# IntelLabs/GKL

Measured on AMD Instinct MI355X. Metric: pairhmm_gcups, higher is better.
Workload: dtype f32

## Files before the change

### gkl_amd/csrc/pairhmm_api.hip

```cpp
#include <hip/hip_runtime.h>
#include <unistd.h>
#include <rccl/rccl.h>
#include <dlfcn.h>

#include <algorithm>
#include <atomic>
#include <cmath>
#include <cstdarg>
#include <cstdio>
#include <cstdlib>
#include <chrono>
#include <condition_variable>
#include <functional>
#include <cstring>
#include <limits>
#include <memory>
#include <mutex>
#include <new>
#include <string>
#include <thread>
#include <deque>
#include <type_traits>
#include <vector>

// ... 353 lines not shown
  static const bool v = server_socket_from_env() != nullptr;
  return v;
}

void* gklhip_host_alloc(size_t bytes) {
  if (client_process()) return malloc(bytes ? bytes : 1);
  void* p = nullptr;
  if (hipHostMalloc(&p, bytes ? bytes : 1, hipHostMallocDefault | hipHostMallocPortable) != hipSuccess) {
    (void)hipGetLastError();
    return nullptr;
  }
  return p;
}

void gklhip_host_free(void* p) {
  if (client_process()) { free(p); return; }
  if (p) (void)hipHostFree(p);
}

static int get_step_times_impl(gklhip_ctx* ctx, int32_t steps_back, float* ms_main, float* ms_fallback, float* ms_total) {
  if (!ctx) return fail(GKLHIP_ERR_INVALID_ARG, "context is NULL");
  if (ctx->remote) return fail(GKLHIP_ERR_UNSUPPORTED, "gklhip_get_step_times: not available on a client context of the PairHMM server");
  std::lock_guard<std::mutex> lock(ctx->mu);
  DevCtx* c = ctx->dev[0];
  if (c->cfg.record_events != 2) return fail(GKLHIP_ERR_INVALID_ARG, "context was not created with record_events = 2");
  if (steps_back < 0 || steps_back >= DevCtx::kEventRing || steps_back >= c->calls)
    return fail(GKLHIP_ERR_INVALID_ARG, "steps_back %d outside the %d recorded calls", steps_back,
                (int)std::min<int64_t>(c->calls, DevCtx::kEventRing));
  HIP_TRY(hipSetDevice(c->device));
  const int slot = (int)((c->calls - 1 - steps_back) % DevCtx::kEventRing);
  hipEvent_t* e = c->ev_ring[slot];
  HIP_TRY(hipEventSynchronize(e[5]));
  float ms = 0;
  HIP_TRY(hipEventElapsedTime(&ms, e[1], e[2])); if (ms_main) *ms_main = ms;
  HIP_TRY(hipEventElapsedTime(&ms, e[3], e[4])); if (ms_fallback) *ms_fallback = c->ring_double[slot] ? 0.f : ms;
  HIP_TRY(hipEventElapsedTime(&ms, e[0], e[5])); if (ms_total) *ms_total = ms;
  return GKLHIP_OK;
}

int gklhip_get_stats(gklhip_ctx* c, gklhip_stats* out) {
  if (!c || !out) return fail(GKLHIP_ERR_INVALID_ARG, "NULL argument");
  std::lock_guard<std::mutex> lock(c->mu);
  *out = c->stats;
  return GKLHIP_OK;
}

static int get_raw_impl(gklhip_ctx* ctx, float* raw32, double* raw64, uint8_t* used64) {
  if (!ctx) return fail(GKLHIP_ERR_INVALID_ARG, "context is NULL");
  if (ctx->remote) return fail(GKLHIP_ERR_UNSUPPORTED, "gklhip_get_raw: the raw sums stay on the PairHMM server (client context)");
  std::lock_guard<std::mutex> lock(ctx->mu);
  int64_t n_fallback = 0;
  bool any = false;
  const std::vector<DevCtx*>& list = ctx->last ? *ctx->last : ctx->dev;
  for (size_t d = 0; d < list.size(); d++) {
    DevCtx* c = list[d];
    if (list.size() > 1 && ctx->bounds[d + 1] == ctx->bounds[d]) continue;
    if (!c->have_last) continue;
    any = true;
    HIP_TRY(hipSetDevice(c->device));
    hipStream_t s = c->last_stream;
    const size_t n = (size_t)c->last_pairs;
    const size_t at = (size_t)ctx->bounds[d] * (size_t)ctx->last_haps;
    if (raw32 && !c->cfg.use_double) HIP_TRY(hipMemcpyAsync(raw32 + at, c->raw32.p, n * 4, hipMemcpyDeviceToHost, s));
    if (raw64) HIP_TRY(hipMemcpyAsync(raw64 + at, c->raw64.p, n * 8, hipMemcpyDeviceToHost, s));
    if (used64) HIP_TRY(hipMemcpyAsync(used64 + at, c->used64.p, n, hipMemcpyDeviceToHost, s));
    int32_t cnt[2] = {0, 0};
    HIP_TRY(hipMemcpyAsync(cnt, c->counters.p, 8, hipMemcpyDeviceToHost, s));
    HIP_TRY(hipStreamSynchronize(s));
    c->stats.n_fallback = c->cfg.use_double ? (int64_t)n : cnt[0];
    n_fallback += c->stats.n_fallback;
  }
  if (!any) return fail(GKLHIP_ERR_INVALID_ARG, "no completed call to read back");
  ctx->stats.n_fallback = n_fallback;
  HIP_TRY(hipSetDevice(ctx->dev[0]->device));
  return GKLHIP_OK;
}

int gklhip_plan_describe(int32_t n_reads, int32_t n_haps, const int64_t* read_off, const int64_t* hap_off,
                         int32_t rows_per_lane, int32_t* lanes_out, int64_t lanes_cap, int32_t* n_groups_out,
                         int32_t* n_long_out) {
  if (n_reads < 0 || n_haps < 0 || !read_off || !hap_off || (rows_per_lane != 4 && rows_per_lane != 8))
    return -fail(GKLHIP_ERR_INVALID_ARG, "bad arguments to gklhip_plan_describe");
  Plan p;
  build_plan(n_reads, n_haps, read_off, hap_off, rows_per_lane, kTargetCols, &p, true);
  if (n_groups_out) *n_groups_out = (int32_t)p.groups.size();
  if (n_long_out) *n_long_out = (int32_t)p.long_reads.size();
  if (lanes_out) {
    const int64_t n = std::min<int64_t>(lanes_cap, (int64_t)p.lanes.size());
    for (int64_t i = 0; i < n; i++) { lanes_out[2 * i] = p.lanes[i].read; lanes_out[2 * i + 1] = p.lanes[i].block; }
  }
  return p.n_chunks;
}

int64_t gklhip_get_table_f32(int which, float* dst, int64_t cap) {
  const HostTables<float>& t = host_tables_f32();
  const std::vector<float>* v = which == 0 ? &t.ph2pr : which == 1 ? &t.mm : which == 2 ? &t.div3 : nullptr;
  if (!v) return -1;
  if (dst) memcpy(dst, v->data(), sizeof(float) * (size_t)std::min<int64_t>(cap, (int64_t)v->size()));
  return (int64_t)v->size();
}
int64_t gklhip_get_table_f64(int which, double* dst, int64_t cap) {
  const HostTables<double>& t = host_tables_f64();
  const std::vector<double>* v = which == 0 ? &t.ph2pr : which == 1 ? &t.mm : which == 2 ? &t.div3 : nullptr;
  if (!v) return -1;
  if (dst) memcpy(dst, v->data(), sizeof(double) * (size_t)std::min<int64_t>(cap, (int64_t)v->size()));
  return (int64_t)v->size();
}

#include "pairhmm_diagnostics.h"

int gklhip_init_devices(const gklhip_config* cfg, const int32_t* devices, int32_t n_devices, gklhip_ctx** out_ctx) { return guarded([&] { return init_devices_impl(cfg, devices, n_devices, out_ctx); }); }
int gklhip_compute_device(gklhip_ctx* c, const gklhip_batch* dev_batch, double* out_dev, void* hip_stream) { return guarded([&] { return compute_device_impl(c, dev_batch, out_dev, hip_stream); }); }
int gklhip_compute(gklhip_ctx* c, const gklhip_batch* hb, double* out_host) { return guarded([&] { return compute_impl(c, hb, out_host); }); }
int gklhip_get_raw(gklhip_ctx* ctx, float* raw32, double* raw64, uint8_t* used64) { return guarded([&] { return get_raw_impl(ctx, raw32, raw64, used64); }); }
int gklhip_get_step_times(gklhip_ctx* ctx, int32_t steps_back, float* ms_main, float* ms_fallback, float* ms_total) { return guarded([&] { return get_step_times_impl(ctx, steps_back, ms_main, ms_fallback, ms_total); }); }
int gklhip_rccl_selftest(int32_t device) { return guarded([&] { return rccl_selftest_impl(device); }); }
int gklhip_init(const gklhip_config* cfg, gklhip_ctx** out_ctx) { return guarded([&] { return init_impl(cfg, out_ctx); }); }

}
```

### gkl_amd/csrc/pairhmm_ctx.h

```cpp
#pragma once

using namespace gklhip;

namespace {
struct EnvSwitches {
  static bool on_unless_zero(const char* name) { const char* v = getenv(name); return !v || atoi(v) != 0; }
  static int integer(const char* name) { const char* v = getenv(name); return v ? atoi(v) : 0; }
  const bool wide_long = on_unless_zero("GKLHIP_WIDE_LONG");
  const bool super_long = on_unless_zero("GKLHIP_SUPER_LONG");
  const bool fused_pairs = on_unless_zero("GKLHIP_FUSED_PAIRS");
  const int64_t fused_max = [] { const char* v = getenv("GKLHIP_FUSED_MAX_PAIRS"); return v ? atoll(v) : -1LL; }();
  const bool xcd_aware = on_unless_zero("GKLHIP_XCD_AWARE");
  const bool timing = getenv("GKLHIP_TIMING") != nullptr;
  const int combine_load = integer("GKL_HIP_COMBINE_LOAD");
  const int target_cols = integer("GKLHIP_TARGET_COLS");
  const int fb_wanted_jobs = integer("GKLHIP_FB_WANTED_JOBS");
  const int plan_blocks = integer("GKLHIP_PLAN_BLOCKS");
  const int finalize_threads = integer("GKL_HIP_FINALIZE_THREADS");
  const int finalize_min = integer("GKL_HIP_FINALIZE_MIN");
  const bool combine = [] { const char* v = getenv("GKL_HIP_COMBINE"); return !(v && v[0] == '0'); }();
  const bool quiet = getenv("GKL_HIP_QUIET") != nullptr;
  const bool one_device_engine = integer("GKL_HIP_DEVICE_ENGINES") == 1;
};
const EnvSwitches g_env;
// ... 6 lines not shown
  char buf[512];
  va_list ap;
  va_start(ap, fmt);
  vsnprintf(buf, sizeof buf, fmt, ap);
  va_end(ap);
  g_err = buf;
  return status;
}

int fail_noexcept(int status, const char* msg) noexcept {
  try { g_err = msg; } catch (...) {}
  return status;
}
template <typename F>
int guarded(F&& body) noexcept {
  try { return body(); }
  catch (const std::bad_alloc&) { return fail_noexcept(GKLHIP_ERR_OOM, "host memory allocation failed"); }
  catch (const std::exception& e) { return fail_noexcept(GKLHIP_ERR_HIP, e.what()); }
  catch (...) { return fail_noexcept(GKLHIP_ERR_HIP, "unexpected C++ exception"); }
}

#define HIP_TRY(expr)                                                                        \
  do {                                                                                       \
    hipError_t e__ = (expr);                                                                 \
    if (e__ != hipSuccess) {                                                                 \
      (void)hipGetLastError();                                                               \
      return fail(e__ == hipErrorOutOfMemory ? GKLHIP_ERR_OOM : GKLHIP_ERR_HIP, "%s: %s",    \
                  #expr, hipGetErrorString(e__));                                            \
    }                                                                                        \
  } while (0)

constexpr size_t kTrimFloor = (size_t)32 << 20;
constexpr int kTrimCalls = 16;
constexpr int kTrimQuiet = 64;
inline bool trim_due(size_t n, size_t cap, int* small_uses, int* since_grow) {
  if (*since_grow < kTrimQuiet) ++*since_grow;
  if (cap <= kTrimFloor || n >= cap / 4) { *small_uses = 0; return false; }
  if (*small_uses < kTrimCalls) ++*small_uses;
  return *small_uses >= kTrimCalls && *since_grow >= kTrimQuiet;
}
struct DevBuf {
  void* p = nullptr;
  size_t cap = 0;
  int small_uses = 0, since_grow = kTrimQuiet;
  int reserve(size_t n) {
    if (n <= cap && !trim_due(n, cap, &small_uses, &since_grow)) return GKLHIP_OK;
    if (n > cap) since_grow = 0;
    small_uses = 0;
    if (p) { (void)hipFree(p); p = nullptr; cap = 0; }
    const size_t want = n + n / 4 + 256;
    HIP_TRY(hipMalloc(&p, want));
    cap = want;
    return GKLHIP_OK;
  }
  void release() { if (p) (void)hipFree(p); p = nullptr; cap = 0; }
  template <typename T> T* as() const { return static_cast<T*>(p); }
};
struct PinBuf {
  void* p = nullptr;
  size_t cap = 0;
  int small_uses = 0, since_grow = kTrimQuiet;
  int reserve(size_t n) {
    if (n <= cap && !trim_due(n, cap, &small_uses, &since_grow)) return GKLHIP_OK;
    if (n > cap) since_grow = 0;
    small_uses = 0;
    if (p) { (void)hipHostFree(p); p = nullptr; cap = 0; }
    const size_t want = n + n / 4 + 256;
    HIP_TRY(hipHostMalloc(&p, want, hipHostMallocDefault));
    cap = want;
    return GKLHIP_OK;
  }
  void release() { if (p) (void)hipHostFree(p); p = nullptr; cap = 0; }
  template <typename T> T* as() const { return static_cast<T*>(p); }
};
}

struct DevCtx {
  gklhip_config cfg;
  int device = 0;
  int n_cus = 256;
  int n_xcds = 8;
  int asm_general = 1;
  int speculate_fp64 = 0;
  int lds_oob_zero = 1;
  hipStream_t stream = nullptr;
  DevBuf tab32, tab64;
  DevTables<float> dt32;
  DevTables<double> dt64;
  PinBuf stage_slot[2];
  DevBuf plan_dev_slot[2];
  hipEvent_t stage_free_slot[2] = {nullptr, nullptr};
  hipEvent_t plan_unused_slot[2] = {nullptr, nullptr};
  hipStream_t upload_stream = nullptr;
  bool upload_eager = false;
  hipStream_t pad_stream = nullptr;
  int plan_slot = 0;
  DevBuf raw32, raw64, used64, counters, stream_buf, out_dev;
  DevBuf lanes_main;
  DevBuf read_fail, lanes2, jobs, jobs_long, fail_order, fail_hist, hap_flags;
  DevBuf batch_dev;
  PinBuf res_pin;
  WorkerPool workers;
  hipStream_t copy_stream = nullptr;
  hipEvent_t policy_done = nullptr, early_copy_done = nullptr;
  hipEvent_t call_done = nullptr;
  bool have_call_done = false;
  static constexpr int kEventRing = 64;
  hipEvent_t ev_ring[kEventRing][6] = {};
  hipEvent_t* ev = ev_ring[0];
  int64_t calls = 0;
  bool ring_double[kEventRing] = {};
  gklhip_stats stats;
  int64_t last_pairs = 0;
  hipStream_t last_stream = nullptr;
  bool have_last = false;
  Plan plan;
  std::vector<PlanLane> long_lanes;
  std::vector<FwdJob> long_jobs;
  std::vector<int64_t> sub_read_off;
  DevBuf carry;
};
```

### gkl_amd/csrc/pairhmm_ctx_lifecycle.h

```cpp
#pragma once

namespace {

std::atomic<int> g_eager_upload_holders{0};

int trim_streams(DevCtx* c) {
  if (!c->copy_stream && !c->pad_stream && (!c->upload_stream || c->upload_eager)) return 0;
  (void)hipSetDevice(c->device);
  for (hipStream_t s : {c->stream, c->copy_stream, c->upload_stream, c->have_last ? c->last_stream : nullptr})
    if (s && hipStreamQuery(s) != hipSuccess) { (void)hipGetLastError(); return 0; }
  int n = 0;
  if (c->copy_stream) { (void)hipStreamDestroy(c->copy_stream); c->copy_stream = nullptr; n++; }
  if (c->pad_stream) { (void)hipStreamDestroy(c->pad_stream); c->pad_stream = nullptr; n++; }
  if (c->upload_stream && !c->upload_eager) { (void)hipStreamDestroy(c->upload_stream); c->upload_stream = nullptr; n++; }
  return n;
}

void dev_done(DevCtx* c) {
  if (!c) return;
  (void)hipSetDevice(c->device);
  if (c->upload_eager) g_eager_upload_holders--;
  if (c->stream) (void)hipStreamSynchronize(c->stream);
  if (c->last_stream && c->have_last) (void)hipStreamSynchronize(c->last_stream);
  for (DevBuf* b : {&c->tab32, &c->tab64, &c->plan_dev_slot[0], &c->plan_dev_slot[1], &c->raw32, &c->raw64, &c->used64,
// ... 4 lines not shown
  c->stage_slot[1].release();
  c->res_pin.release();
  if (c->policy_done) (void)hipEventDestroy(c->policy_done);
  if (c->early_copy_done) (void)hipEventDestroy(c->early_copy_done);
  if (c->call_done) (void)hipEventDestroy(c->call_done);
  if (c->copy_stream) { (void)hipStreamSynchronize(c->copy_stream); (void)hipStreamDestroy(c->copy_stream); }
  for (auto& set : c->ev_ring)
    for (auto& e : set) if (e) (void)hipEventDestroy(e);
  for (int k = 0; k < 2; k++) {
    if (c->stage_free_slot[k]) (void)hipEventDestroy(c->stage_free_slot[k]);
    if (c->plan_unused_slot[k]) (void)hipEventDestroy(c->plan_unused_slot[k]);
  }
  if (c->upload_stream) { (void)hipStreamSynchronize(c->upload_stream); (void)hipStreamDestroy(c->upload_stream); }
  if (c->pad_stream) (void)hipStreamDestroy(c->pad_stream);
  if (c->stream) (void)hipStreamDestroy(c->stream);
  delete c;
}

int dev_init(const gklhip_config& cfg, int dev, int ndev, DevCtx** out) {
  *out = nullptr;
  if (dev < 0 || dev >= ndev) return fail(GKLHIP_ERR_INVALID_ARG, "device %d of %d", dev, ndev);
  HIP_TRY(hipSetDevice(dev));
  {
    static const char* sched = getenv("GKL_HIP_SCHEDULE");
    if (sched && *sched) {
      const unsigned f = strcmp(sched, "yield") == 0 ? hipDeviceScheduleYield : strcmp(sched, "blocking") == 0 ? hipDeviceScheduleBlockingSync
                         : strcmp(sched, "spin") == 0 ? hipDeviceScheduleSpin : hipDeviceScheduleAuto;
      (void)hipSetDeviceFlags(f);
      (void)hipGetLastError();
    }
  }
  hipDeviceProp_t prop;
  HIP_TRY(hipGetDeviceProperties(&prop, dev));
  if (strncmp(prop.gcnArchName, "gfx950", 6) != 0)
    return fail(GKLHIP_ERR_NO_DEVICE, "device %d is %s; this library is built for gfx950 only", dev, prop.gcnArchName);
  DevCtx* c = new (std::nothrow) DevCtx();
  if (!c) return fail(GKLHIP_ERR_OOM, "context allocation failed");
  c->cfg = cfg;
  c->device = dev;
  c->n_cus = std::max(1, prop.multiProcessorCount);
  {
    int xccs = 0;
    if (hipDeviceGetAttribute(&xccs, hipDeviceAttributeNumberOfXccs, dev) != hipSuccess) { (void)hipGetLastError(); xccs = 8; }
    c->n_xcds = std::max(1, std::min(xccs, 64));
  }
  memset(&c->stats, 0, sizeof c->stats);
  int rc = GKLHIP_OK;
  auto bail = [&](int status) { dev_done(c); return status; };
  if (hipStreamCreateWithFlags(&c->stream, hipStreamNonBlocking) != hipSuccess) return bail(fail(GKLHIP_ERR_HIP, "hipStreamCreate failed"));
  {
    static std::mutex mu;
    static std::vector<int> checked;
    std::lock_guard<std::mutex> l(mu);
    if ((int)checked.size() <= dev) checked.resize((size_t)dev + 1, 0);
    static std::vector<int> oob_checked;
    if ((int)oob_checked.size() <= dev) oob_checked.resize((size_t)dev + 1, 0);
    if (checked[(size_t)dev] == 0 || oob_checked[(size_t)dev] == 0) {
      uint32_t* d_out = nullptr;
      uint32_t h_out[3] = {1u, 1u, 1u};
      if (hipMalloc(reinterpret_cast<void**>(&d_out), 12) != hipSuccess) return bail(fail(GKLHIP_ERR_OOM, "hipMalloc failed"));
      float f_den; double d_den;
      { const uint32_t fb = 1u; memcpy(&f_den, &fb, 4); const uint64_t db = 0x0000000100000001ull; memcpy(&d_den, &db, 8); }
      bool ok = hipMemsetAsync(d_out, 0, 12, c->stream) == hipSuccess;
      hipLaunchKernelGGL(flush_selftest_kernel, dim3(1), dim3(1), 0, c->stream, d_out, f_den, d_den);
      hipLaunchKernelGGL(lds_oob_selftest_kernel, dim3(1024), dim3(256), 0, c->stream, d_out + 2);
      hipLaunchKernelGGL((lds_oob_selftest_big_kernel<78 * 256, 512>), dim3(4 * 2 * (unsigned)c->n_cus), dim3(512), 0, c->stream, d_out + 2);
      hipLaunchKernelGGL((lds_oob_selftest_big_kernel<128 * 256, 256>), dim3(4 * (unsigned)c->n_cus), dim3(256), 0, c->stream, d_out + 2);
      ok = ok && hipGetLastError() == hipSuccess && hipMemcpyAsync(h_out, d_out, 12, hipMemcpyDeviceToHost, c->stream) == hipSuccess &&
           hipStreamSynchronize(c->stream) == hipSuccess;
      (void)hipFree(d_out);
      if (!ok) { (void)hipGetLastError(); return bail(fail(GKLHIP_ERR_HIP, "the start-up self-tests could not run on device %d", dev)); }
      checked[(size_t)dev] = h_out[0] == 0u && h_out[1] == 0u ? 1 : -1;
      oob_checked[(size_t)dev] = h_out[2] == 0u ? 1 : -1;
      if (oob_checked[(size_t)dev] < 0)
        fprintf(stderr, "[gklhip] pairhmm: LDS reads beyond the allocation do not return 0 on device %d (%08x): the fp32 general steps stay in C++\n", dev, h_out[2]);
    }
    if (checked[(size_t)dev] < 0)
      return bail(fail(GKLHIP_ERR_HIP, "this library was built without the denormal-flush flags its kernels depend on (gkl_amd/csrc/Makefile: HIPFLAGS)"));
    c->lds_oob_zero = oob_checked[(size_t)dev] > 0 ? 1 : 0;
  }
  {
    const char* ag = getenv("GKLHIP_ASM_GENERAL");
    c->asm_general = ag ? (atoi(ag) != 0) : 1;
    const char* sp = getenv("GKLHIP_SPECULATE_FP64");
    c->speculate_fp64 = sp ? (atoi(sp) != 0) : 0;
    const char* sf = getenv("GKLHIP_SELFTEST_FAIL");
    if (sf && strcmp(sf, "lds_oob") == 0) {
      c->lds_oob_zero = 0;
      fprintf(stderr, "[gklhip] pairhmm: GKLHIP_SELFTEST_FAIL=lds_oob: the fp32 general steps stay in C++ for this context\n");
    }
  }
  if (g_eager_upload_holders.fetch_add(1) == 0) {
    if (hipStreamCreateWithFlags(&c->upload_stream, hipStreamNonBlocking) != hipSuccess) { g_eager_upload_holders--; return bail(fail(GKLHIP_ERR_HIP, "hipStreamCreate failed")); }
    c->upload_eager = true;
  } else {
    g_eager_upload_holders--;
  }
  if (const char* v = getenv("GKL_HIP_EAGER_STREAMS")) {
    const int k = atoi(v);
    if (k >= 7) { if (aux_streams(c) != GKLHIP_OK) return bail(GKLHIP_ERR_HIP); }
    else for (int i = 0; i < k; i++) { hipStream_t d = nullptr; (void)hipStreamCreateWithFlags(&d, hipStreamNonBlocking); }
  }
  for (int k = 0; k < 2; k++)
    if (hipEventCreateWithFlags(&c->stage_free_slot[k], hipEventDisableTiming) != hipSuccess ||
        hipEventCreateWithFlags(&c->plan_unused_slot[k], hipEventDisableTiming) != hipSuccess)
      return bail(fail(GKLHIP_ERR_HIP, "hipEventCreate failed"));
  if (hipEventCreateWithFlags(&c->policy_done, hipEventDisableTiming) != hipSuccess ||
      hipEventCreateWithFlags(&c->early_copy_done, hipEventDisableTiming) != hipSuccess ||
      hipEventCreateWithFlags(&c->call_done, hipEventDisableTiming) != hipSuccess)
    return bail(fail(GKLHIP_ERR_HIP, "hipEventCreate failed"));
  for (int k = 0; k < 2; k++)
    if (hipEventRecord(c->stage_free_slot[k], c->stream) != hipSuccess || hipEventRecord(c->plan_unused_slot[k], c->stream) != hipSuccess)
      return bail(fail(GKLHIP_ERR_HIP, "hipEventRecord failed"));
  {
    const int sets = c->cfg.record_events == 2 ? DevCtx::kEventRing : 1;
    for (int k = 0; k < sets; k++)
      for (auto& e : c->ev_ring[k])
        if (hipEventCreate(&e) != hipSuccess) return bail(fail(GKLHIP_ERR_HIP, "hipEventCreate failed"));
  }
  if ((rc = upload_tables(c, host_tables_f32(), &c->tab32, &c->dt32))) return bail(rc);
  if ((rc = upload_tables(c, host_tables_f64(), &c->tab64, &c->dt64))) return bail(rc);
  *out = c;
  return GKLHIP_OK;
}

}
```

### gkl_amd/csrc/pairhmm_device_pass.h

```cpp
#pragma once

namespace {

int aux_streams(DevCtx* c) {
  if (!c->upload_stream) HIP_TRY(hipStreamCreateWithFlags(&c->upload_stream, hipStreamNonBlocking));
  if (!c->copy_stream) {
    HIP_TRY(hipStreamCreateWithFlags(&c->copy_stream, hipStreamNonBlocking));
    if (!c->pad_stream) HIP_TRY(hipStreamCreateWithFlags(&c->pad_stream, hipStreamNonBlocking));
  }
  return GKLHIP_OK;
}

template <typename T>
int upload_tables(DevCtx* c, const HostTables<T>& h, DevBuf* buf, DevTables<T>* dt) {
  const size_t n = (size_t)kQuals * 2 + kMmEntries;
  int st = buf->reserve(n * sizeof(T));
  if (st) return st;
  T* base = buf->as<T>();
  {
    T* pin = nullptr;
    HIP_TRY(hipHostMalloc(reinterpret_cast<void**>(&pin), n * sizeof(T), hipHostMallocDefault));
    memcpy(pin, h.ph2pr.data(), kQuals * sizeof(T));
    memcpy(pin + kQuals, h.div3.data(), kQuals * sizeof(T));
    memcpy(pin + 2 * kQuals, h.mm.data(), kMmEntries * sizeof(T));
// ... 163 lines not shown
    int64_t blocks = 0;
    for (int r = 0; r < n_reads; r++) {
      const int nb = blocks_for((int)(read_off[r + 1] - read_off[r]), rpl);
      if (nb <= kLanes) blocks += nb;
    }
    const int64_t chunks = std::max<int64_t>(1, (blocks + kLanes - 1) / kLanes);
    const int64_t groups = std::min<int64_t>(n_haps, std::max<int64_t>((total_cols + kTargetCols - 1) / kTargetCols,
                                                                        (4096 + chunks - 1) / chunks));
    return chunks * groups;
  };
  if (jobs_at(kRplF32) * load >= 2048 || max_len > 4 * kLanes - 1) return kRplF32;
  if (jobs_at(4) * load >= 1024 || max_len > 2 * kLanes - 1) return 4;
  return 2;
}

void launch_pair_policy_two_step(const FwdArgs<double>& d, const PairPolicyArgs& q, int rows, int fma, int64_t n_pairs, int32_t* list, hipStream_t s) {
  hipLaunchKernelGGL(pairhmm_pair_flag_kernel, dim3((unsigned)((n_pairs + 255) / 256)), dim3(256), 0, s, q, (int32_t)n_pairs, list);
  const dim3 grid((unsigned)std::max<int64_t>(256, n_pairs / 2)), block(64);
  if (fma) {
    if (rows == 2)      hipLaunchKernelGGL((pairhmm_pair_recompute_kernel<2, true>), grid, block, 0, s, d, q, list);
    else if (rows == 4) hipLaunchKernelGGL((pairhmm_pair_recompute_kernel<4, true>), grid, block, 0, s, d, q, list);
    else                hipLaunchKernelGGL((pairhmm_pair_recompute_kernel<kRplF64, true>), grid, block, 0, s, d, q, list);
  } else {
    if (rows == 2)      hipLaunchKernelGGL((pairhmm_pair_recompute_kernel<2, false>), grid, block, 0, s, d, q, list);
    else if (rows == 4) hipLaunchKernelGGL((pairhmm_pair_recompute_kernel<4, false>), grid, block, 0, s, d, q, list);
    else                hipLaunchKernelGGL((pairhmm_pair_recompute_kernel<kRplF64, false>), grid, block, 0, s, d, q, list);
  }
}
void launch_main_f32(const FwdArgs<float>& a, int rpl_main, int fma, int n_blocks, hipStream_t s) {
  if (rpl_main == 2)      launch_stream<float, 2>(a, fma, n_blocks, s);
  else if (rpl_main == 4) launch_stream<float, 4>(a, fma, n_blocks, s);
  else                    launch_stream<float, kRplF32>(a, fma, n_blocks, s);
}
void launch_pair_policy(const FwdArgs<double>& d, const PairPolicyArgs& q, int rows, int fma, int64_t n_pairs, hipStream_t s) {
  const dim3 grid((unsigned)n_pairs), block(64);
  if (fma) {
    if (rows == 2)      hipLaunchKernelGGL((pairhmm_pair_policy_kernel<2, true>), grid, block, 0, s, d, q);
    else if (rows == 4) hipLaunchKernelGGL((pairhmm_pair_policy_kernel<4, true>), grid, block, 0, s, d, q);
    else                hipLaunchKernelGGL((pairhmm_pair_policy_kernel<kRplF64, true>), grid, block, 0, s, d, q);
  } else {
    if (rows == 2)      hipLaunchKernelGGL((pairhmm_pair_policy_kernel<2, false>), grid, block, 0, s, d, q);
    else if (rows == 4) hipLaunchKernelGGL((pairhmm_pair_policy_kernel<4, false>), grid, block, 0, s, d, q);
    else                hipLaunchKernelGGL((pairhmm_pair_policy_kernel<kRplF64, false>), grid, block, 0, s, d, q);
  }
}

void launch_pair_fused(const FwdArgs<float>& f, const FwdArgs<double>& d, const PairPolicyArgs& q, int rows, int fma, int64_t n_pairs,
                       hipStream_t s, bool speculate = false) {
  if (speculate) {
    const dim3 grid((unsigned)n_pairs), block(128);
    if (fma) hipLaunchKernelGGL((pairhmm_pair_spec_kernel<kRplF64, true>), grid, block, 0, s, f, d, q);
    else     hipLaunchKernelGGL((pairhmm_pair_spec_kernel<kRplF64, false>), grid, block, 0, s, f, d, q);
    return;
  }
  const dim3 grid((unsigned)n_pairs), block(64);
  if (rows <= 4) {
    if (fma) hipLaunchKernelGGL((pairhmm_pair_fused_kernel<4, true>), grid, block, 0, s, f, d, q);
    else     hipLaunchKernelGGL((pairhmm_pair_fused_kernel<4, false>), grid, block, 0, s, f, d, q);
    return;
  }
  if (fma) hipLaunchKernelGGL((pairhmm_pair_fused_kernel<kRplF64, true>), grid, block, 0, s, f, d, q);
  else     hipLaunchKernelGGL((pairhmm_pair_fused_kernel<kRplF64, false>), grid, block, 0, s, f, d, q);
}

int run_device(DevCtx* c, const gklhip_batch* db, double* out_dev, int finalize_mode, hipStream_t s, bool inline_host,
               SmallLaunch* defer = nullptr) {
  const int n_reads = db->n_reads, n_haps = db->n_haps;
  const int64_t n_pairs = (int64_t)n_reads * n_haps;
  gklhip_stats& st = c->stats;
  memset(&st, 0, sizeof st);
  st.n_pairs = n_pairs;
  c->have_last = false;
  if (n_pairs == 0) return GKLHIP_OK;
  const bool use_double = c->cfg.use_double != 0;
  const int fma = c->cfg.fma_mode != 0;

  const auto t_plan0 = std::chrono::steady_clock::now();
  Plan& plan = c->plan;
  const int rpl64 = kRplF64Jobs;
  const int load_env = g_env.combine_load;
  const int load = !defer ? 1 : load_env > 0 ? load_env : std::max(1, g_host_calls_in_flight.load(std::memory_order_relaxed) / 2);
  const int rpl_main = use_double ? rpl64 : pick_f32_rpl(c->cfg.rows_per_lane, n_reads, n_haps, db->read_off, db->hap_off, load);
  const int target_cols_env = g_env.target_cols;
  build_plan(n_reads, n_haps, db->read_off, db->hap_off, rpl_main, target_cols_env > 0 ? target_cols_env : kTargetCols, &plan);
  std::vector<PlanLane>& long_lanes = c->long_lanes;
  std::vector<FwdJob>& long_jobs = c->long_jobs;
  long_lanes.clear(); long_jobs.clear();
  const std::vector<int32_t>& long_main = plan.long_reads;
  const int n_long_main = (int)long_main.size();
  for (int32_t r : long_main) { long_lanes.resize(long_lanes.size() + kLanes, PlanLane{-1, 0}); long_lanes[long_lanes.size() - kLanes] = PlanLane{r, 0}; }
  int n_long64 = 0;
  if (!use_double && plan.max_read_len > kLanes * kRplF64Jobs - 1)
    for (int r = 0; r < n_reads; r++)
      if (blocks_for((int)(db->read_off[r + 1] - db->read_off[r]), kRplF64Jobs) > kLanes) {
        long_lanes.resize(long_lanes.size() + kLanes, PlanLane{-1, 0});
        long_lanes[long_lanes.size() - kLanes] = PlanLane{r, 0};
        n_long64++;
      }
  for (int i = 0; i < n_long_main; i++)
    for (const PlanGroup& g : plan.groups) long_jobs.push_back(FwdJob{i, g.hap_begin, g.hap_end, 0});
  int carry_len = 0;
  for (const PlanGroup& g : plan.groups) {
    const int last = g.hap_end - 1;
    carry_len = std::max(carry_len, plan.hap_pos[last] + plan.hap_len[last] - plan.hap_pos[g.hap_begin] + 3 * kLanes);
  }
  carry_len = (carry_len + 63) / 64 * 64;
  const size_t rl = (size_t)db->read_off[n_reads], hl = (size_t)db->hap_off[n_haps];
  const PlanLayout L = layout_for(plan, n_reads, n_haps, long_lanes.size(), long_jobs.size(), inline_host ? rl : 0, inline_host ? hl : 0);

  int rc;
  const int slot = c->plan_slot ^= 1;
  PinBuf& stage = c->stage_slot[slot];
  DevBuf& plan_dev = c->plan_dev_slot[slot];
  HIP_TRY(hipEventSynchronize(c->stage_free_slot[slot]));
  if (L.total > stage.cap || L.total > plan_dev.cap) HIP_TRY(hipEventSynchronize(c->plan_unused_slot[slot]));
  if ((rc = stage.reserve(L.total))) return rc;
  if ((rc = plan_dev.reserve(L.total))) return rc;
  unsigned char* hs = stage.as<unsigned char>();
  memcpy(hs + L.place_chunk, plan.place_chunk.data(), (size_t)n_reads * 4);
  memcpy(hs + L.place_lane, plan.place_lane.data(), (size_t)n_reads);
  memcpy(hs + L.chunk_used, plan.chunk_used.data(), (size_t)plan.n_chunks);
  memcpy(hs + L.groups, plan.groups.data(), plan.groups.size() * sizeof(PlanGroup));
  memcpy(hs + L.hap_len, plan.hap_len.data(), (size_t)n_haps * 4);
  memcpy(hs + L.hap_pos, plan.hap_pos.data(), (size_t)n_haps * 4);
  memcpy(hs + L.hap_pos_flat, plan.hap_pos_flat.data(), (size_t)n_haps * 4);
  memcpy(hs + L.hap_orig, plan.hap_orig.data(), (size_t)n_haps * 4);
  memcpy(hs + L.hap_sidx, plan.hap_sidx.data(), (size_t)n_haps * 4);
  memcpy(hs + L.hap_group, plan.hap_group.data(), (size_t)n_haps * 4);
  memcpy(hs + L.hap_src, plan.hap_src.data(), (size_t)n_haps * 4);
  {
    float* y32 = reinterpret_cast<float*>(hs + L.y0_32);
    double* y64 = reinterpret_cast<double*>(hs + L.y0_64);
    const float i32 = host_tables_f32().initial_constant;
    const double i64 = host_tables_f64().initial_constant;
    for (int k = 0; k < n_haps; k++) {
      y32[k] = i32 / (float)plan.hap_len[k];
      y64[k] = i64 / (double)plan.hap_len[k];
    }
  }
  memcpy(hs + L.read_off, db->read_off, (size_t)(n_reads + 1) * 8);
  if (!long_lanes.empty()) memcpy(hs + L.long_lanes, long_lanes.data(), long_lanes.size() * sizeof(PlanLane));
  if (!long_jobs.empty()) memcpy(hs + L.long_jobs, long_jobs.data(), long_jobs.size() * sizeof(FwdJob));
  {
    int32_t lc[4] = {(int32_t)long_jobs.size(), n_long_main, n_long64, 0};
    memcpy(hs + L.long_count, lc, sizeof lc);
  }
  unsigned char* dp = plan_dev.as<unsigned char>();
  gklhip_batch dbi = *db;
  if (inline_host) {
    const uint8_t* srcs[5] = {db->read_bases, db->read_quals, db->ins_gop, db->del_gop, db->gcp};
    for (int i = 0; i < 5; i++) memcpy(hs + L.batch + i * L.batch_stride, srcs[i], rl);
    memcpy(hs + L.batch + 5 * L.batch_stride, db->hap_bases, hl);
    unsigned char* d = dp + L.batch;
    dbi.read_bases = d; dbi.read_quals = d + L.batch_stride; dbi.ins_gop = d + 2 * L.batch_stride;
    dbi.del_gop = d + 3 * L.batch_stride; dbi.gcp = d + 4 * L.batch_stride; dbi.hap_bases = d + 5 * L.batch_stride;
    uint32_t* sg = reinterpret_cast<uint32_t*>(hs + L.stream);
    uint32_t* sf = reinterpret_cast<uint32_t*>(hs + L.stream_flat);
    uint8_t* hn = hs + L.has_n;
    for (int k = 0; k < n_haps; k++) {
      const uint8_t* src = db->hap_bases + plan.hap_src[k];
      const int len = plan.hap_len[k], pg = plan.hap_pos[k], pf = plan.hap_pos_flat[k];
      bool has_n = false;
      for (int col = 0; col < len; col++) {
        const uint8_t bb = src[col];
        const uint32_t e = bb == 'C' ? 1u : bb == 'T' ? 2u : bb == 'G' ? 3u : bb == 'N' ? 4u : 0u;
        sg[pg + col] = e; sf[pf + col] = e;
        has_n |= bb == 'N';
// ... 349 lines not shown
```

### gkl_amd/csrc/pairhmm_plan.cpp

```cpp
#include "pairhmm_plan.h"

#include <algorithm>
#include <cstdlib>
#include <numeric>

namespace gklhip {

namespace {
constexpr int kLanes = 64;
constexpr int kWantedJobs = 4096;
}

void build_plan(int n_reads, int n_haps, const int64_t* read_off, const int64_t* hap_off,
                int rows_per_lane, int target_cols, Plan* out, bool want_lanes) {
  Plan& p = *out;
  p.rows_per_lane = rows_per_lane;
  p.n_chunks = 0;
  p.n_stream = p.n_stream_flat = 0;
  p.useful_rows = 0;
  p.max_read_len = p.max_hap_len = 0;
  p.groups.clear(); p.long_reads.clear(); p.lanes.clear(); p.chunk_used.clear();

  p.hap_len.resize(n_haps);
  p.hap_pos.resize(n_haps);
  p.hap_pos_flat.resize(n_haps);
  p.hap_orig.resize(n_haps);
  p.hap_sidx.resize(n_haps);
  p.hap_group.resize(n_haps);
  p.hap_src.resize(n_haps);
  int64_t total_cols = 0;
  std::iota(p.hap_orig.begin(), p.hap_orig.end(), 0);
  std::stable_sort(p.hap_orig.begin(), p.hap_orig.end(), [&](int32_t a, int32_t b) {
    return hap_off[a + 1] - hap_off[a] < hap_off[b + 1] - hap_off[b];
  });
  for (int k = 0; k < n_haps; k++) {
    const int h = p.hap_orig[k];
    const int len = (int)(hap_off[h + 1] - hap_off[h]);
    p.hap_len[k] = len;
    p.hap_sidx[h] = k;
    p.max_hap_len = std::max(p.max_hap_len, len);
    total_cols += len + 1;
  }
  if (target_cols < 256) target_cols = 256;
  int n_groups = (int)((total_cols + target_cols - 1) / target_cols);
  bool equal_split = true, graded = false;
  if (rows_per_lane > 0) {
    int64_t blocks = 0;
    {
      int shift = -1;
      for (int b = 0; b < 8; b++) if ((1 << b) == rows_per_lane) shift = b;
      const int long_from = kLanes * rows_per_lane;
      for (int r = 0; r < n_reads; r++) {
        const int R = (int)(read_off[r + 1] - read_off[r]);
        p.max_read_len = std::max(p.max_read_len, R);
        if (R < long_from) blocks += shift >= 0 ? (R + rows_per_lane) >> shift : blocks_for(R, rows_per_lane);
      }
    }
    const int64_t chunks_est = std::max<int64_t>(1, (blocks + kLanes - 1) / kLanes);
    static const int wanted_env = [] { const char* v = getenv("GKLHIP_WANTED_JOBS"); return v ? atoi(v) : 0; }();
    const int64_t slots = kWantedJobs, chunks_hi = chunks_est + chunks_est / 100 + 1;
    const int64_t wanted = wanted_env > 0 ? wanted_env : (chunks_est <= 650 || total_cols <= 4 * (int64_t)target_cols ? 3 * slots : slots);
    int64_t by_jobs = std::min<int64_t>((wanted + chunks_est - 1) / chunks_est, n_haps);
    if (chunks_hi * by_jobs > slots && chunks_hi * by_jobs * 10 <= slots * 13) by_jobs = std::max<int64_t>(1, slots / chunks_hi);
    graded = chunks_hi * by_jobs > slots;
    if (by_jobs >= n_groups) n_groups = (int)by_jobs;
    else equal_split = false;
  }
  n_groups = std::max(1, std::min(n_groups, n_haps));
  std::vector<int64_t> want;
  if (equal_split || total_cols < 3 * (int64_t)target_cols) {
    const int64_t per_group = (total_cols + n_groups - 1) / n_groups;
    want.assign((size_t)n_groups, per_group);
    if (graded && equal_split && n_groups >= 4)
      for (int i = 0; i < n_groups; i++)
        want[(size_t)i] = std::max<int64_t>(1, (int64_t)((double)per_group * (1.35 - 0.7 * (double)i / (double)(n_groups - 1))));
  } else {
    const int64_t tail[4] = {target_cols / 2, target_cols / 4, target_cols / 8, target_cols / 8};
    const int64_t head = total_cols - target_cols;
    const int n_big = (int)std::max<int64_t>(1, (head + target_cols / 2) / target_cols);
    want.assign((size_t)n_big, (head + n_big - 1) / n_big);
    want.insert(want.end(), tail, tail + 4);
  }
  {
    int h = 0;
    size_t gi = 0;
    while (h < n_haps) {
      PlanGroup g;
      g.hap_begin = h;
      g.stream_begin = p.n_stream;
      g.pad_ = 0;
      int64_t cols = 0;
      const bool last = gi + 1 >= want.size();
      const int64_t share = want[std::min(gi, want.size() - 1)];
      do {
        p.hap_pos[h] = p.n_stream;
        p.hap_pos_flat[h] = p.n_stream_flat;
        p.n_stream_flat += p.hap_len[h] + 1;
        p.hap_group[h] = (int32_t)p.groups.size();
        p.hap_src[h] = (int32_t)hap_off[p.hap_orig[h]];
        p.n_stream += p.hap_len[h] + 1;
        cols += p.hap_len[h] + 1;
        h++;
      } while (h < n_haps && (last || cols + (p.hap_len[h] + 1) / 2 < share));
      g.hap_end = h;
      p.n_stream += kLanes;
      p.groups.push_back(g);
      gi++;
    }
  }

  p.n_stream_flat += kLanes;

  if (rows_per_lane <= 0)
    for (int r = 0; r < n_reads; r++)
      p.max_read_len = std::max(p.max_read_len, (int)(read_off[r + 1] - read_off[r]));
  p.place_chunk.resize((size_t)n_reads);
  p.place_lane.resize((size_t)n_reads);
  if (rows_per_lane <= 0 || n_reads == 0) return;
  static thread_local std::vector<int32_t> order;
  static thread_local PackScratch scratch;
  order.clear();
  const int long_from = kLanes * rows_per_lane;
  if (p.max_read_len < long_from) {
    order.resize((size_t)n_reads);
    std::iota(order.begin(), order.end(), 0);
  } else {
    for (int r = 0; r < n_reads; r++) {
      if ((int)(read_off[r + 1] - read_off[r]) < long_from) order.push_back(r);
      else { p.long_reads.push_back(r); p.place_chunk[r] = -1; p.place_lane[r] = 0; }
    }
  }
  p.n_chunks = pack_reads_place(order.data(), (int)order.size(), read_off, rows_per_lane,
                                (int)std::max<size_t>(order.size(), 1), p.place_chunk.data(), p.place_lane.data(),
                                &p.chunk_used, &p.useful_rows, &scratch);
  if (want_lanes) expand_lanes(p, n_reads, read_off, &p.lanes);
}

void expand_lanes(const Plan& p, int n_reads, const int64_t* read_off, std::vector<PlanLane>* lanes) {
  lanes->assign((size_t)p.n_chunks * kLanes, PlanLane{-1, 0});
  for (int r = 0; r < n_reads; r++) {
    if (p.place_chunk[r] < 0) continue;
    const int nb = blocks_for((int)(read_off[r + 1] - read_off[r]), p.rows_per_lane);
    PlanLane* dst = lanes->data() + (size_t)p.place_chunk[r] * kLanes + p.place_lane[r];
    for (int b = 0; b < nb; b++) dst[b] = PlanLane{r, b};
  }
}

int pack_reads_place(const int32_t* order_in, int n, const int64_t* read_off, int rows_per_lane, int window,
                     int32_t* place_chunk, uint8_t* place_lane, std::vector<uint8_t>* chunk_used,
                     int64_t* useful_rows, PackScratch* sc) {
  const int rpl = rows_per_lane;
  if (window < 1) window = 1;
  int shift = -1;
  for (int b = 0; b < 8; b++) if ((1 << b) == rpl) shift = b;
  sc->need_of.resize((size_t)n);
  int64_t rows = 0;
  for (int i = 0; i < n; i++) {
    const int32_t r = order_in[i];
    const int R = (int)(read_off[r + 1] - read_off[r]);
    sc->need_of[i] = (uint8_t)(shift >= 0 ? (R + rpl) >> shift : blocks_for(R, rpl));
    rows += R;
  }
  if (useful_rows) *useful_rows += rows;
  const int wcap = std::min(n, window);
  sc->sorted.resize((size_t)wcap);
  sc->sorted_need.resize((size_t)wcap);
  const uint8_t* need_of = sc->need_of.data();
  int chunks_total = 0;
  for (int w0 = 0; w0 < n; w0 += window) {
    const int cnt = std::min(window, n - w0);
    int32_t bucket[kLanes + 2] = {0};
    for (int i = 0; i < cnt; i++) bucket[need_of[w0 + i]]++;
    int32_t start[kLanes + 2];
    int acc = 0;
    for (int c = kLanes; c >= 1; c--) { start[c] = acc; acc += bucket[c]; }
    for (int i = 0; i < cnt; i++) {
      const int at = start[need_of[w0 + i]]++;
      sc->sorted[at] = order_in[w0 + i];
      sc->sorted_need[at] = need_of[w0 + i];
    }
    int32_t head[kLanes + 1];
    for (int c = 0; c <= kLanes; c++) head[c] = -1;
    uint64_t open_sizes = 0;
    const size_t base = chunk_used->size();
    sc->next.clear();
    for (int i = 0; i < cnt; i++) {
      const int32_t r = sc->sorted[i];
      const int nb = sc->sorted_need[i];
      const uint64_t fits = nb <= 63 ? open_sizes >> (nb - 1) : 0;
      int chunk, c;
      if (!fits) {
        chunk = (int)sc->next.size();
        sc->next.push_back(-1);
        chunk_used->push_back(0);
        c = kLanes;
      } else {
        c = nb + __builtin_ctzll(fits);
        chunk = head[c];
        head[c] = sc->next[chunk];
        if (head[c] < 0) open_sizes &= ~(1ull << (c - 1));
      }
      uint8_t& used = (*chunk_used)[base + (size_t)chunk];
      place_chunk[r] = (int32_t)(base + (size_t)chunk);
      place_lane[r] = used;
      used = (uint8_t)(used + nb);
      const int left = c - nb;
      if (left > 0) { sc->next[chunk] = head[left]; head[left] = chunk; open_sizes |= 1ull << (left - 1); }
    }
    chunks_total += (int)sc->next.size();
  }
  return chunks_total;
}

int pack_reads_windowed(const int32_t* order_in, int n, const int64_t* read_off, int rows_per_lane,
                        int window, std::vector<PlanLane>* lanes, int64_t* useful_rows) {
  const int rpl = rows_per_lane;
  if (window < 1) window = 1;
  int chunks_total = 0;
  int shift = -1;
  for (int b = 0; b < 8; b++) if ((1 << b) == rpl) shift = b;
  std::vector<uint8_t> need_of((size_t)n);
  int64_t need_sum = 0;
  for (int i = 0; i < n; i++) {
    const int32_t r = order_in[i];
    const int R = (int)(read_off[r + 1] - read_off[r]);
    need_of[i] = (uint8_t)(shift >= 0 ? (R + rpl) >> shift : blocks_for(R, rpl));
    need_sum += need_of[i];
    if (useful_rows) *useful_rows += R;
  }
  {
    const size_t want = lanes->size() + (size_t)(need_sum + need_sum / 8 + 2 * kLanes);
    if (lanes->capacity() < want) lanes->reserve(std::max(want, 2 * lanes->capacity()));
  }
  std::vector<int32_t> sorted((size_t)std::min(n, window));
  std::vector<uint8_t> sorted_need((size_t)std::min(n, window));
  std::vector<int32_t> next;
  std::vector<int32_t> used;
  for (int w0 = 0; w0 < n; w0 += window) {
    const int cnt = std::min(window, n - w0);
    int32_t bucket[kLanes + 2] = {0};
    for (int i = 0; i < cnt; i++) bucket[need_of[w0 + i]]++;
    int32_t start[kLanes + 2];
    int acc = 0;
    for (int c = kLanes; c >= 1; c--) { start[c] = acc; acc += bucket[c]; }
    for (int i = 0; i < cnt; i++) {
      const int at = start[need_of[w0 + i]]++;
      sorted[at] = order_in[w0 + i];
      sorted_need[at] = need_of[w0 + i];
    }
    int32_t head[kLanes + 1];
    for (int c = 0; c <= kLanes; c++) head[c] = -1;
    next.clear();
    used.clear();
    const size_t base = lanes->size();
    for (int i = 0; i < cnt; i++) {
      const int32_t r = sorted[i];
      const int nb = sorted_need[i];
      int c = nb;
      while (c <= kLanes && head[c] < 0) c++;
      int chunk;
      if (c > kLanes) {
        chunk = (int)used.size();
        used.push_back(0);
        next.push_back(-1);
        lanes->resize(base + (size_t)(chunk + 1) * kLanes, PlanLane{-1, 0});
        c = kLanes;
      } else {
        chunk = head[c];
        head[c] = next[chunk];
// ... 14 lines not shown
```

### gkl_amd/csrc/pairhmm_plan.h

```cpp
#pragma once
#include <cstdint>
#include <vector>

namespace gklhip {

struct PlanLane {
  int32_t read;
  int32_t block;
};

struct PlanGroup {
  int32_t hap_begin, hap_end, stream_begin, pad_;
};

struct Plan {
  int rows_per_lane = 0;
  int n_chunks = 0;
  std::vector<int32_t> place_chunk;
  std::vector<uint8_t> place_lane;
  std::vector<uint8_t> chunk_used;
  std::vector<PlanLane> lanes;
  std::vector<PlanGroup> groups;
  std::vector<int32_t> hap_len;
  std::vector<int32_t> hap_pos;
  std::vector<int32_t> hap_pos_flat;
  std::vector<int32_t> hap_orig;
  std::vector<int32_t> hap_sidx;
  std::vector<int32_t> hap_group;
  std::vector<int32_t> hap_src;
  int32_t n_stream = 0;
  int32_t n_stream_flat = 0;
  std::vector<int32_t> long_reads;
  int64_t useful_rows = 0;
  int max_read_len = 0;
  int max_hap_len = 0;
};

inline int blocks_for(int R, int rpl) { return (R + rpl) / rpl; }

void build_plan(int n_reads, int n_haps, const int64_t* read_off, const int64_t* hap_off,
                int rows_per_lane, int target_cols, Plan* out, bool want_lanes = false);

void expand_lanes(const Plan& p, int n_reads, const int64_t* read_off, std::vector<PlanLane>* lanes);

int pack_reads_windowed(const int32_t* order, int n, const int64_t* read_off, int rows_per_lane,
                        int window, std::vector<PlanLane>* lanes, int64_t* useful_rows);

struct PackScratch {
  std::vector<uint8_t> need_of, sorted_need;
  std::vector<int32_t> sorted, next;
};
int pack_reads_place(const int32_t* order, int n, const int64_t* read_off, int rows_per_lane, int window,
                     int32_t* place_chunk, uint8_t* place_lane, std::vector<uint8_t>* chunk_used,
                     int64_t* useful_rows, PackScratch* scratch);

}
```

Before: 4761.

## Pack reads into chunks with bounded exact-fill search before best-fit

```diff
diff --git a/gkl_amd/csrc/pairhmm_api.hip b/gkl_amd/csrc/pairhmm_api.hip
--- a/gkl_amd/csrc/pairhmm_api.hip
+++ b/gkl_amd/csrc/pairhmm_api.hip
@@ -459,7 +459,7 @@
   if (n_reads < 0 || n_haps < 0 || !read_off || !hap_off || (rows_per_lane != 4 && rows_per_lane != 8))
     return -fail(GKLHIP_ERR_INVALID_ARG, "bad arguments to gklhip_plan_describe");
   Plan p;
-  build_plan(n_reads, n_haps, read_off, hap_off, rows_per_lane, kTargetCols, &p, true);
+  build_plan(n_reads, n_haps, read_off, hap_off, rows_per_lane, kTargetCols, &p, true, EnvSwitches::on_unless_zero("GKLHIP_EXACT_FIT"));
   if (n_groups_out) *n_groups_out = (int32_t)p.groups.size();
   if (n_long_out) *n_long_out = (int32_t)p.long_reads.size();
   if (lanes_out) {
diff --git a/gkl_amd/csrc/pairhmm_ctx.h b/gkl_amd/csrc/pairhmm_ctx.h
--- a/gkl_amd/csrc/pairhmm_ctx.h
+++ b/gkl_amd/csrc/pairhmm_ctx.h
@@ -112,6 +112,7 @@
   int n_xcds = 8;
   int asm_general = 1;
   int speculate_fp64 = 0;
+  int exact_fit = 1;
   int lds_oob_zero = 1;
   hipStream_t stream = nullptr;
   DevBuf tab32, tab64;
diff --git a/gkl_amd/csrc/pairhmm_ctx_lifecycle.h b/gkl_amd/csrc/pairhmm_ctx_lifecycle.h
--- a/gkl_amd/csrc/pairhmm_ctx_lifecycle.h
+++ b/gkl_amd/csrc/pairhmm_ctx_lifecycle.h
@@ -110,6 +110,7 @@
   {
     const char* ag = getenv("GKLHIP_ASM_GENERAL");
     c->asm_general = ag ? (atoi(ag) != 0) : 1;
+    c->exact_fit = EnvSwitches::on_unless_zero("GKLHIP_EXACT_FIT") ? 1 : 0;
     const char* sp = getenv("GKLHIP_SPECULATE_FP64");
     c->speculate_fp64 = sp ? (atoi(sp) != 0) : 0;
     const char* sf = getenv("GKLHIP_SELFTEST_FAIL");
diff --git a/gkl_amd/csrc/pairhmm_device_pass.h b/gkl_amd/csrc/pairhmm_device_pass.h
--- a/gkl_amd/csrc/pairhmm_device_pass.h
+++ b/gkl_amd/csrc/pairhmm_device_pass.h
@@ -269,7 +269,8 @@
   const int load = !defer ? 1 : load_env > 0 ? load_env : std::max(1, g_host_calls_in_flight.load(std::memory_order_relaxed) / 2);
   const int rpl_main = use_double ? rpl64 : pick_f32_rpl(c->cfg.rows_per_lane, n_reads, n_haps, db->read_off, db->hap_off, load);
   const int target_cols_env = g_env.target_cols;
-  build_plan(n_reads, n_haps, db->read_off, db->hap_off, rpl_main, target_cols_env > 0 ? target_cols_env : kTargetCols, &plan);
+  build_plan(n_reads, n_haps, db->read_off, db->hap_off, rpl_main, target_cols_env > 0 ? target_cols_env : kTargetCols, &plan,
+             false, c->exact_fit != 0);
   std::vector<PlanLane>& long_lanes = c->long_lanes;
   std::vector<FwdJob>& long_jobs = c->long_jobs;
   long_lanes.clear(); long_jobs.clear();
diff --git a/gkl_amd/csrc/pairhmm_plan.cpp b/gkl_amd/csrc/pairhmm_plan.cpp
--- a/gkl_amd/csrc/pairhmm_plan.cpp
+++ b/gkl_amd/csrc/pairhmm_plan.cpp
@@ -12,7 +12,7 @@
 }
 
 void build_plan(int n_reads, int n_haps, const int64_t* read_off, const int64_t* hap_off,
-                int rows_per_lane, int target_cols, Plan* out, bool want_lanes) {
+                int rows_per_lane, int target_cols, Plan* out, bool want_lanes, bool exact_fit) {
   Plan& p = *out;
   p.rows_per_lane = rows_per_lane;
   p.n_chunks = 0;
@@ -132,7 +132,7 @@
   }
   p.n_chunks = pack_reads_place(order.data(), (int)order.size(), read_off, rows_per_lane,
                                 (int)std::max<size_t>(order.size(), 1), p.place_chunk.data(), p.place_lane.data(),
-                                &p.chunk_used, &p.useful_rows, &scratch);
+                                &p.chunk_used, &p.useful_rows, &scratch, exact_fit);
   if (want_lanes) expand_lanes(p, n_reads, read_off, &p.lanes);
 }
 
@@ -146,9 +146,49 @@
   }
 }
 
+namespace {
+
+bool exact_fill(int32_t* left, uint64_t* avail, int s, int mx, int* budget, uint8_t* picked, int* n_picked) {
+  const int top = std::min(s, mx);
+  uint64_t cand = *avail & (top >= 64 ? ~0ull : (1ull << top) - 1);
+  while (cand) {
+    const int c = 64 - __builtin_clzll(cand);
+    cand &= ~(1ull << (c - 1));
+    if (--*budget < 0) return false;
+    if (--left[c] == 0) *avail &= ~(1ull << (c - 1));
+    picked[(*n_picked)++] = (uint8_t)c;
+    if (c == s || exact_fill(left, avail, s - c, c, budget, picked, n_picked)) return true;
+    (*n_picked)--;
+    if (left[c]++ == 0) *avail |= 1ull << (c - 1);
+  }
+  return false;
+}
+
+int best_fit_chunks(const int32_t* bucket) {
+  int32_t open[kLanes + 1] = {0};
+  uint64_t open_sizes = 0;
+  int chunks = 0;
+  for (int nb = kLanes; nb >= 1; nb--) {
+    for (int32_t k = 0; k < bucket[nb]; k++) {
+      const uint64_t fits = nb <= 63 ? open_sizes >> (nb - 1) : 0;
+      int c = kLanes;
+      if (!fits) chunks++;
+      else {
+        c = nb + __builtin_ctzll(fits);
+        if (--open[c] == 0) open_sizes &= ~(1ull << (c - 1));
+      }
+      const int rest = c - nb;
+      if (rest > 0) { open[rest]++; open_sizes |= 1ull << (rest - 1); }
+    }
+  }
+  return chunks;
+}
+
+}
+
 int pack_reads_place(const int32_t* order_in, int n, const int64_t* read_off, int rows_per_lane, int window,
                      int32_t* place_chunk, uint8_t* place_lane, std::vector<uint8_t>* chunk_used,
-                     int64_t* useful_rows, PackScratch* sc) {
+                     int64_t* useful_rows, PackScratch* sc, bool exact_fit) {
   const int rpl = rows_per_lane;
   if (window < 1) window = 1;
   int shift = -1;
@@ -184,7 +224,53 @@
     uint64_t open_sizes = 0;
     const size_t base = chunk_used->size();
     sc->next.clear();
-    for (int i = 0; i < cnt; i++) {
+    int first = 0;
+    if (exact_fit && cnt == n) {
+      int32_t left[kLanes + 1], pos[kLanes + 1], deferred[kLanes + 1] = {0};
+      for (int c = 1; c <= kLanes; c++) { left[c] = bucket[c]; pos[c] = start[c] - bucket[c]; }
+      left[0] = 0;
+      uint64_t avail = 0;
+      for (int c = 1; c <= kLanes; c++) if (left[c] > 0) avail |= 1ull << (c - 1);
+      uint8_t picked[kLanes];
+      int n_deferred = 0;
+      for (int lead = kLanes; lead >= 1; lead--) {
+        while (left[lead] > 0) {
+          if (--left[lead] == 0) avail &= ~(1ull << (lead - 1));
+          int n_picked = 0, budget = 64;
+          if (lead < kLanes && !exact_fill(left, &avail, kLanes - lead, lead, &budget, picked, &n_picked)) {
+            deferred[lead] += 1 + left[lead]; n_deferred += 1 + left[lead];
+            left[lead] = 0;
+            avail &= ~(1ull << (lead - 1));
+            break;
+          }
+          const int32_t chunk = (int32_t)chunk_used->size();
+          uint8_t used = 0;
+          for (int k = -1; k < n_picked; k++) {
+            const int nb = k < 0 ? lead : picked[k];
+            const int32_t r = sc->sorted[pos[nb]++];
+            place_chunk[r] = chunk;
+            place_lane[r] = used;
+            used = (uint8_t)(used + nb);
+          }
+          chunk_used->push_back(used);
+        }
+      }
+      const int closed = (int)(chunk_used->size() - base);
+      if (closed + best_fit_chunks(deferred) <= best_fit_chunks(bucket)) {
+        first = cnt - n_deferred;
+        int at = cnt;
+        for (int c = 1; c <= kLanes; c++)
+          for (int32_t k = deferred[c] - 1; k >= 0; k--) {
+            --at;
+            sc->sorted[at] = sc->sorted[pos[c] + k];
+            sc->sorted_need[at] = (uint8_t)c;
+          }
+        sc->next.assign((size_t)closed, -1);
+      } else {
+        chunk_used->resize(base);
+      }
+    }
+    for (int i = first; i < cnt; i++) {
       const int32_t r = sc->sorted[i];
       const int nb = sc->sorted_need[i];
       const uint64_t fits = nb <= 63 ? open_sizes >> (nb - 1) : 0;
diff --git a/gkl_amd/csrc/pairhmm_plan.h b/gkl_amd/csrc/pairhmm_plan.h
--- a/gkl_amd/csrc/pairhmm_plan.h
+++ b/gkl_amd/csrc/pairhmm_plan.h
@@ -39,7 +39,7 @@
 inline int blocks_for(int R, int rpl) { return (R + rpl) / rpl; }
 
 void build_plan(int n_reads, int n_haps, const int64_t* read_off, const int64_t* hap_off,
-                int rows_per_lane, int target_cols, Plan* out, bool want_lanes = false);
+                int rows_per_lane, int target_cols, Plan* out, bool want_lanes = false, bool exact_fit = true);
 
 void expand_lanes(const Plan& p, int n_reads, const int64_t* read_off, std::vector<PlanLane>* lanes);
 
@@ -52,6 +52,6 @@
 };
 int pack_reads_place(const int32_t* order, int n, const int64_t* read_off, int rows_per_lane, int window,
                      int32_t* place_chunk, uint8_t* place_lane, std::vector<uint8_t>* chunk_used,
-                     int64_t* useful_rows, PackScratch* scratch);
+                     int64_t* useful_rows, PackScratch* scratch, bool exact_fit = false);
 
 }
```

Result: no change. 4769 (median of 6 runs) (+0.2%).
